# JediZ/PDE-based-image-processing

Hardware: AMD Instinct MI355X
Metric: SOR iterations/sec (3840x2160 flow) (higher is better)
Workload: dtype f32

## Files before the change

### include/pdeip.h

```cpp
#ifndef PDEIP_H
#define PDEIP_H

#ifdef __cplusplus
extern "C" {
#endif

#define PDEIP_OK 0
#define PDEIP_ERR_ARG 1
#define PDEIP_ERR_SOLVER 2
#define PDEIP_ERR_UNSUPPORTED 3
#define PDEIP_ERR_DEVICE 4
#define PDEIP_ERR_NOMEM 5

#define PDEIP_MODE_EXACT_ORDER 0
#define PDEIP_MODE_RED_BLACK 1
#define PDEIP_MODE_LINE_SCAN 2

#define PDEIP_SOLVER_SOR 1
#define PDEIP_SOLVER_ALR 2

const char *pdeip_version(void);
const char *pdeip_last_error(void);
int pdeip_set_mode(int mode);
int pdeip_get_mode(void);
int pdeip_set_device(int device_id);
int pdeip_set_devices(int n, const int *ids);
int pdeip_get_devices(int *ids, int capacity);
int pdeip_release(void);
int pdeip_last_launch_count(void);
int pdeip_workspace_generation(void);
int pdeip_persist_error(void);
int pdeip_debug_raise_abort(void);
int pdeip_debug_persist_order(int B, int T, int affine, int *table);
enum { PDEIP_PLAN_ELIN4 = 0, PDEIP_PLAN_LLIN4, PDEIP_PLAN_DISP4, PDEIP_PLAN_PDE4, PDEIP_PLAN_PDE8, PDEIP_PLAN_DISPSYM4 };
enum { PDEIP_PLAN_INFO = 11, PDEIP_PLAN_RECORD = 9 };
int pdeip_debug_plan_sor(int model, int nrows, int ncols, int nframes, int iter, int mode, int aligned16, int has_dst, int num_cus,
                         int rb2_slots, int rbp_slots, int *info, int *records, int capacity);
enum { PDEIP_PLAN_ALR_ELIN4 = 0, PDEIP_PLAN_ALR_LLIN4, PDEIP_PLAN_ALR_LLIN8, PDEIP_PLAN_ALR_DISP4, PDEIP_PLAN_ALR_PDE4, PDEIP_PLAN_ALR_PDE8 };
enum { PDEIP_PLAN_ALR_INFO = 12, PDEIP_PLAN_ALR_PASS = 20 };
int pdeip_debug_plan_alr(int model, int nrows, int ncols, int nframes, int iter, int mode, int *info, int *passes);
int pdeip_debug_rcp_check(unsigned long long *counts);
int pdeip_profile_enable(int on);
int pdeip_profile_read(double *elapsed_ms, int *sweep_launches);


int pdeip_oflow_sor_elin4(const float *U, const float *V, const float *M, const float *Cu,
                          const float *Cv, const float *Du, const float *Dv, const float *wW,
                          const float *wN, const float *wE, const float *wS, int nrows, int ncols,
                          int nframes_coef, int iter, float omega, int solver, float *U_out,
                          float *V_out, float *RU, float *RV);

int pdeip_oflow_sor_llin4(const float *U, const float *V, const float *dU, const float *dV,
                          const float *M, const float *Cu, const float *Cv, const float *Du,
                          const float *Dv, const float *wW, const float *wN, const float *wE,
                          const float *wS, int nrows, int ncols, int nframes_coef, int iter,
                          float omega, int solver, float *dU_out, float *dV_out, float *RU,
                          float *RV);

int pdeip_oflow_sor_llin8(const float *U, const float *V, const float *dU, const float *dV,
                          const float *M, const float *Cu, const float *Cv, const float *Du,
                          const float *Dv, const float *wW, const float *wNW, const float *wN,
                          const float *wNE, const float *wE, const float *wSE, const float *wS,
                          const float *wSW, int nrows, int ncols, int nframes_coef, int iter,
                          float omega, int solver, float *dU_out, float *dV_out, float *RU,
                          float *RV);

int pdeip_oflow_lhs_elin4(const float *U, const float *V, const float *M, const float *Du,
                          const float *Dv, const float *wW, const float *wN, const float *wE,
                          const float *wS, int nrows, int ncols, int nframes_coef, float *AU,
                          float *AV);

int pdeip_oflow_lhs_llin4(const float *U, const float *V, const float *dU, const float *dV,
                          const float *M, const float *Du, const float *Dv, const float *wW,
                          const float *wN, const float *wE, const float *wS, int nrows, int ncols,
                          int nframes_coef, float *AU, float *AV);

int pdeip_disp_sor_llin4(const float *U, const float *dU, const float *Cu, const float *Du,
                         const float *wW, const float *wN, const float *wE, const float *wS,
                         int nrows, int ncols, int iter, float omega, int solver, float *dU_out,
                         float *RU);

int pdeip_disp_sor_llin_sym4(const float *U0, const float *dU0, const float *Cu0, const float *Du0, const float *wW0,
// ... 409 lines not shown
```

### pde-based-image-processing_amd/capi.py

```python
import ctypes
import os

HERE = os.path.dirname(os.path.abspath(__file__))
LIB_PATH = os.environ.get("PDEIP_LIB") or os.path.join(HERE, "libpdeip.so")

PDEIP_OK = 0
PDEIP_ERR_ARG = 1
PDEIP_ERR_SOLVER = 2
PDEIP_ERR_UNSUPPORTED = 3
PDEIP_ERR_DEVICE = 4
PDEIP_ERR_NOMEM = 5
MODE_EXACT_ORDER = 0
MODE_RED_BLACK = 1
SEG_SURFACE, SEG_GREEDY, SEG_INVERSE = 0, 1, 2
MODE_LINE_SCAN = 2

_P = ctypes.c_void_p
_I = ctypes.c_int
_F = ctypes.c_float


class PdeipError(RuntimeError):

    def __init__(self, code, message):
# ... 113 lines not shown
                                 ctypes.c_ulonglong, _P, _P, _P, _P, _P],
    "pdeip_seg_label_dev": [_P, _P, _I, _I, _I, _P],
    "pdeip_seg_label": [_P, _I, _I, _I, _P],
    "pdeip_bwlabel_dev": [_P, _P, _I, _I, _I, _P, _P, _P, _I],
    "pdeip_bwlabel": [_P, _I, _I, _I, _P, _P, _P, _I],
    "pdeip_largest_component_dev": [_P, _P, _I, _I, _I, _F, _F, _P, _P, _P],
    "pdeip_largest_component": [_P, _I, _I, _I, _F, _F, _P, _P, _P],
    "pdeip_generate_seeds": [_P, _P, _I, _I, _I, ctypes.c_double, _P, _I, _I, _I, ctypes.c_double, ctypes.c_double, ctypes.c_ulonglong, _P, _P, _P,
                             _P, _P, _P],
    "pdeip_disp_segmentation": [_P, _I, _I, _P, _I, _P, _P, ctypes.c_ulonglong, _P, _P, _P, _P],
    "pdeip_nanmedfilt2_dev": [_P, _P, _I, _I, _I, _P],
    "pdeip_nanmedfilt2": [_P, _I, _I, _I, _P],
    "pdeip_sparse_pyramid": [_P, _I, _I, ctypes.c_double, ctypes.c_double, _I, _P, _P, _P],
    "pdeip_generate_seeds_sparse": [_P, _P, _I, _I, _I, ctypes.c_double, _P, _I, _I, _I, ctypes.c_double, ctypes.c_double, ctypes.c_ulonglong, _P,
                                    _P, _P, _P, _P, _P],
    "pdeip_region_competition_sparse": [_P, _P, _I, _I, _I, _I, _I, ctypes.c_double, _F, _I, ctypes.c_double, ctypes.c_double, ctypes.c_double,
                                        ctypes.c_ulonglong, _P, _P, _P, _P, _P],
    "pdeip_disp_segmentation_sparse": [_P, _I, _I, _P, _I, _P, _P, ctypes.c_ulonglong, _P, _P, _P, _P],
    "pdeip_flow2color_dev": [_P, _P, _P, _I, _I, ctypes.c_double, _I, _P, _P, _P],
    "pdeip_flow2color": [_P, _P, _I, _I, ctypes.c_double, _I, _P, _P, _P],
    "pdeip_flow_errors_dev": [_P, _P, _P, _P, _P, _P, _I, _I, _P, _P, _P],
    "pdeip_flow_errors": [_P, _P, _P, _P, _P, _I, _I, _P, _P, _P],
    "pdeip_disp_crosscheck_dev": [_P, _P, _P, _I, _I, ctypes.c_double, _P, _P, _P, _P],
    "pdeip_disp_crosscheck": [_P, _P, _I, _I, ctypes.c_double, _P, _P, _P, _P],
    "pdeip_flow_crosscheck_dev": [_P, _P, _P, _P, _P, _I, _I, ctypes.c_double, ctypes.c_double, _P, _P, _P],
    "pdeip_flow_crosscheck": [_P, _P, _P, _P, _I, _I, ctypes.c_double, ctypes.c_double, _P, _P, _P],
    "pdeip_nan_resize_dev": [_P, _P, _I, _I, _I, _I, _I, ctypes.c_double, _P],
    "pdeip_inpaint_meanfill_dev": [_P, _P, _I, _I, _I, _P],
    "pdeip_tv4_inpaint_assemble_dev": [_P, _P, _P, _P, _I, ctypes.c_double, _I, _I, _I, _F] + [_P] * 6,
    "pdeip_inpaint_merge_dev": [_P, _P, _P, _I, _I, _I, _P, _P],
    "pdeip_tv_inpaint4_dev": [_P, _P, _I, _I, _I, _P, _I, _P, _P, _P],
    "pdeip_tv_inpaint4": [_P, _I, _I, _I, _P, _I, _P, _P, _P],
    "pdeip_flow_splat_dev": [_P, _P, _P, _P, _P, _I, _I, _I, ctypes.c_double, _P, _P, _P],
    "pdeip_interp_blend_dev": [_P, _P, _P, _I, _P, _P, _P, _P, _I, _I, ctypes.c_double, _P, _P],
    "pdeip_flow_interpolate_dev": [_P, _P, _P, _I, _P, _P, _P, _P, _I, _I, ctypes.c_double, _P, _P, _P, _P, _P],
    "pdeip_flow_interpolate": [_P, _P, _I, _P, _P, _P, _P, _I, _I, ctypes.c_double, _P, _P, _P, _P, _P],
    "pdeip_gauss_taps": [ctypes.c_double, _P, _I, ctypes.POINTER(ctypes.c_int)],
    "pdeip_gauss": [_P, _I, _I, _I, ctypes.c_double, _P],
    "pdeip_gauss_dev": [_P, _P, _I, _I, _I, ctypes.c_double, _P],
    "pdeip_structure_tensor_dev": [_P, _P, _I, _I, _I, ctypes.c_double, ctypes.c_double, _P],
    "pdeip_st_weights_dev": [_P, _P, _I, _I, _P, ctypes.c_double, _P, _P],
    "pdeip_st_weights_padded_dev": [_P, _P, _I, _I, _P, ctypes.c_double, _P, _P],
    "pdeip_st_pad_dev": [_P, _P, _I, _I, _I, _P, _P],
    "pdeip_st_crop_dev": [_P, _P, _I, _I, _I, _P],
    "pdeip_diffusion8": [_P, _I, _I, _I, _P, _P],
    "pdeip_diffusion8_dev": [_P, _P, _I, _I, _I, _P, _P],
    "pdeip_set_mode": [_I],
    "pdeip_get_mode": [],
    "pdeip_set_device": [_I],
    "pdeip_set_devices": [_I, ctypes.POINTER(ctypes.c_int)],
    "pdeip_get_devices": [ctypes.POINTER(ctypes.c_int), _I],
    "pdeip_release": [],
    "pdeip_last_launch_count": [],
    "pdeip_workspace_generation": [],
    "pdeip_persist_error": [],
    "pdeip_debug_persist_order": [_I, _I, _I, ctypes.POINTER(ctypes.c_int)],
    "pdeip_debug_raise_abort": [],
    "pdeip_debug_plan_sor": [_I] * 11 + [ctypes.POINTER(ctypes.c_int), ctypes.POINTER(ctypes.c_int), _I],
    "pdeip_debug_plan_alr": [_I] * 6 + [ctypes.POINTER(ctypes.c_int), ctypes.POINTER(ctypes.c_int)],
    "pdeip_debug_rcp_check": [ctypes.POINTER(ctypes.c_ulonglong)],
    "pdeip_profile_enable": [_I],
    "pdeip_profile_read": [ctypes.POINTER(ctypes.c_double), ctypes.POINTER(ctypes.c_int)],
}
STRING_FUNCS = ("pdeip_version", "pdeip_last_error")

_lib = None


def load():
    global _lib
    if _lib is not None:
        return _lib
    if not os.path.exists(LIB_PATH):
        raise PdeipError(PDEIP_ERR_DEVICE,
                         "libpdeip.so is not built (%s). Run `python __graft_entry__.py build`; "
                         "there is no CPU fallback." % LIB_PATH)
    try:
        import torch
    except ImportError:
        pass
    try:
        lib = ctypes.CDLL(LIB_PATH)
    except OSError as exc:
        raise PdeipError(PDEIP_ERR_DEVICE, "cannot load %s: %s" % (LIB_PATH, exc)) from exc
    for name, argtypes in SIGNATURES.items():
        fn = getattr(lib, name)
        fn.argtypes = argtypes
        fn.restype = ctypes.c_int
    for name in STRING_FUNCS:
        fn = getattr(lib, name)
        fn.argtypes = []
        fn.restype = ctypes.c_char_p
    _lib = lib
    return lib


def last_error():
    return load().pdeip_last_error().decode("utf-8", "replace")


def check(rc):
    if rc != PDEIP_OK:
        raise PdeipError(rc, last_error())


_fn_cache = {}
# ... 43 lines not shown
```

### pde-based-image-processing_amd/csrc/pdeip_ctx.hip

```cpp
#include "pdeip_ctx.hpp"

namespace pdeip {

Context g;
thread_local ThreadState tls;

int set_err(int code, const char *fmt, ...)
{
    va_list ap;
    va_start(ap, fmt);
    vsnprintf(tls.err, sizeof tls.err, fmt, ap);
    va_end(ap);
    return code;
}

SweepTimer::SweepTimer(hipStream_t stream, int total_launches) : s(stream), total(total_launches)
{
    if (!g.profile) return;
    hipStreamCaptureStatus capturing = hipStreamCaptureStatusNone;
    if (hipStreamIsCapturing(s, &capturing) != hipSuccess || capturing != hipStreamCaptureStatusNone) return;
    std::lock_guard<std::mutex> lock(g.ev_mutex);
    if (g.n_ev >= Context::MAX_EV) return;
    if (g.n_ev == g.n_ev_created) {
        if (hipEventCreateWithFlags(&g.ev[g.n_ev][0], hipEventDisableSystemFence) != hipSuccess) return;
// ... 220 lines not shown
}

}

using namespace pdeip;

extern "C" const char *pdeip_version(void) { return "pdeip-mi355x 0.2 (gfx950)"; }
extern "C" const char *pdeip_last_error(void) { return tls.err; }
extern "C" int pdeip_set_mode(int mode)
{
    RC(check_mode("pdeip_set_mode", mode));
    g.mode = mode;
    mode_set_explicitly = true;
    return PDEIP_OK;
}
extern "C" int pdeip_get_mode(void)
{
    read_env_once();
    return g.mode;
}
extern "C" int pdeip_set_devices(int n, const int *ids)
{
    int have = 0;
    HIPCHK(hipGetDeviceCount(&have));
    if (n < 1 || n > MAX_DEVICES || !ids) return set_err(PDEIP_ERR_ARG, "pdeip_set_devices: need 1..%d device ids", MAX_DEVICES);
    for (int k = 0; k < n; k++) {
        if (ids[k] < 0 || ids[k] >= have || ids[k] >= MAX_DEVICES)
            return set_err(PDEIP_ERR_ARG, "pdeip_set_devices: no device %d (have %d)", ids[k], have);
        for (int j = 0; j < k; j++)
            if (ids[j] == ids[k]) return set_err(PDEIP_ERR_ARG, "pdeip_set_devices: device %d named twice", ids[k]);
    }
    for (int k = 0; k < n; k++) g.group[k] = ids[k];
    g.ngroup = n;
    devices_set_explicitly = true;
    return PDEIP_OK;
}
extern "C" int pdeip_set_device(int device_id) { return pdeip_set_devices(1, &device_id); }
extern "C" int pdeip_get_devices(int *ids, int capacity)
{
    read_env_once();
    for (int k = 0; k < g.ngroup && k < capacity; k++)
        if (ids) ids[k] = g.group[k];
    return g.ngroup;
}
extern "C" int pdeip_release(void)
{
    int cur = 0;
    const bool have_cur = hipGetDevice(&cur) == hipSuccess;
    for (int k = 0; k < MAX_DEVICES; k++) release_device(&g.devs[k]);
    if (have_cur) (void)hipSetDevice(cur);
    return PDEIP_OK;
}
extern "C" int pdeip_last_launch_count(void) { return tls.last_launches; }
extern "C" int pdeip_workspace_generation(void) { return g.ws_generation; }
extern "C" int pdeip_persist_error(void)
{
    bool bad = false;
    int cur = 0;
    const bool have_cur = hipGetDevice(&cur) == hipSuccess;
    for (int k = 0; k < MAX_DEVICES; k++) {
        DeviceState *d = &g.devs[k];
        if (d->device < 0) continue;
        if (d->persist_used && d->ws[WS_CTL]) {
            HIPCHK(hipSetDevice(d->device));
            unsigned word = 0;
            HIPCHK(hipDeviceSynchronize());
            HIPCHK(hipMemcpy(&word, d->ws[WS_CTL], sizeof word, hipMemcpyDeviceToHost));
            if (word != 0) {
                bad = true;
                HIPCHK(hipMemset(d->ws[WS_CTL], 0, sizeof(unsigned)));
            }
            d->persist_used = false;
        }
        if (d->abort_latched) bad = true;
        d->abort_latched = false;
    }
    if (have_cur) (void)hipSetDevice(cur);
    if (bad) return set_err(PDEIP_ERR_DEVICE, "persistent exact-order kernel: a dependency wait timed out (results are invalid)");
    return PDEIP_OK;
}
extern "C" int pdeip_debug_raise_abort(void)
{
    RC(use_device());
    float *ctl = nullptr;
    RC(ws_get(WS_CTL, 16, &ctl));
    const unsigned one = 1u;
    HIPCHK(hipDeviceSynchronize());
    HIPCHK(hipMemcpy(ctl, &one, sizeof one, hipMemcpyHostToDevice));
    cur_dev()->persist_used = true;
    return PDEIP_OK;
}

extern "C" int pdeip_profile_enable(int on)
{
    g.profile = (on != 0);
    g.n_ev = 0;
    return PDEIP_OK;
}
extern "C" int pdeip_profile_read(double *elapsed_ms, int *sweep_launches)
{
    double ms = 0.0;
    int launches = 0;
    for (int k = 0; k < g.n_ev; k++) {
        HIPCHK(hipEventSynchronize(g.ev[k][1]));
        float t = 0.0f;
        HIPCHK(hipEventElapsedTime(&t, g.ev[k][0], g.ev[k][1]));
// ... 9 lines not shown
```

### pde-based-image-processing_amd/csrc/pdeip_ctx.hpp

```cpp
#pragma once
#include "../../include/pdeip.h"

#include <hip/hip_runtime.h>
#include <hip/hip_ext.h>

#include <atomic>
#include <cstdarg>
#include <cstdio>
#include <cstdlib>
#include <cstring>
#include <map>
#include <mutex>
#include <vector>

namespace pdeip {

enum { WS_AUX0 = 0, WS_AUX1, WS_PING, WS_ARENA, WS_CTL, WS_ORDER, WS_ALR, WS_ALR_T, WS_TV, WS_SMALL, WS_MAIL, WS_PACK, WS_DRIVER, WS_LEX, WS_LS, WS_RANSAC, WS_SEG_STAGE, WS_SEG, WS_SEG_RC, WS_CCL, WS_SEEDS, WS_SELECT, WS_GAC, WS_RANSAC_BATCH, WS_FLOWVIZ, WS_CROSSCHECK, WS_INTERP, WS_GAUSS, WS_STENSOR, WS_NSLOT };

constexpr int MAX_DEVICES = 16;

struct DeviceState {
    int device = -1;
    void *ws[WS_NSLOT] = {};
    size_t ws_bytes[WS_NSLOT] = {};
    int num_cus = 0;
    bool persist_used = false;
    bool abort_latched = false;
    std::map<const void *, size_t> lds_opt_in;
    std::map<const void *, int> resident_waves;
    hipStream_t worker_stream = nullptr;
    void reset_caches()
    {
        persist_used = false;
    }
};

struct ThreadState {
    char err[512] = "";
    int last_launches = 0;
    int dev_slot = -1;
};
extern thread_local ThreadState tls;

struct Context {
    int mode = PDEIP_MODE_EXACT_ORDER;
    std::atomic<int> ws_generation{0};
    int rb_tj = 0;
    bool env_read = false;
    int ngroup = 1;
    int group[MAX_DEVICES] = {0};
    DeviceState devs[MAX_DEVICES];
    bool profile = false;
    static constexpr int MAX_EV = 4096;
    hipEvent_t ev[MAX_EV][2];
    int ev_launches[MAX_EV];
    int n_ev = 0, n_ev_created = 0;
    std::mutex ev_mutex;
};
extern Context g;

int set_err(int code, const char *fmt, ...);

#define HIPCHK(expr)                                                                                       \
    do {                                                                                                   \
        hipError_t e_ = (expr);                                                                            \
        if (e_ != hipSuccess) return ::pdeip::set_err(PDEIP_ERR_DEVICE, "%s failed: %s", #expr, hipGetErrorString(e_)); \
    } while (0)

#define RC(expr)             \
    do {                     \
        int rc_ = (expr);    \
        if (rc_) return rc_; \
    } while (0)

#define NONNULL(who, p)                                                                                \
    do {                                                                                               \
        if ((p) == nullptr) return ::pdeip::set_err(PDEIP_ERR_ARG, "%s: argument '%s' is NULL", who, #p); \
    } while (0)

struct SweepTimer {
    hipStream_t s;
    int slot = -1;
    int total = 0;
    explicit SweepTimer(hipStream_t stream, int total_launches = 0);
    hipEvent_t start_for(int launch) const { return (slot >= 0 && total > 0 && launch == 0) ? g.ev[slot][0] : nullptr; }
    hipEvent_t stop_for(int launch) const { return (slot >= 0 && total > 0 && launch == total - 1) ? g.ev[slot][1] : nullptr; }
    void stop(int launches);
};

template <class... KArgs, class... Args>
inline void launch_timed(void (*kernel)(KArgs...), dim3 grid, dim3 block, size_t lds, hipStream_t s, hipEvent_t start, hipEvent_t stop, Args... args)
{
// ... 45 lines not shown
```

### pde-based-image-processing_amd/csrc/pdeip_multi.hip

```cpp
#include "pdeip_ctx.hpp"

#include <thread>

using namespace pdeip;

namespace pdeip {

constexpr int OVERLAP_SLABS = 6;
struct SlabPlan {
    int nslabs = 1, halo = 0, nrows = 0;
    bool overlap = false;
    int c0[MAX_DEVICES], c1[MAX_DEVICES], lo[MAX_DEVICES], hi[MAX_DEVICES], dev[MAX_DEVICES];
};

int multi_plan(int ncols, int halo, SlabPlan *plan)
{
    read_env_once();
    int want = g.ngroup;
    const int virt = env_int("PDEIP_VIRTUAL_SLABS", 0);
    if (virt > want) want = virt;
    plan->overlap = false;
    if (want == 1 && virt <= 0 && env_int("PDEIP_HOST_OVERLAP", 1) != 0 && (long)ncols * plan->nrows >= (1L << 21) && ncols / OVERLAP_SLABS >= 4 * (halo + 1)) {
        want = OVERLAP_SLABS;
        plan->overlap = true;
// ... 98 lines not shown
    int vthreads = g.ngroup == 1 ? env_int("PDEIP_VIRTUAL_THREADS", plan.overlap ? 2 : 0) : 0;
    if (vthreads > plan.nslabs) vthreads = plan.nslabs;
    if (vthreads > MAX_DEVICES / 2) vthreads = MAX_DEVICES / 2;
    if (vthreads > 1) {
        nth = vthreads;
        for (int ti = 0; ti < nth; ti++) {
            devs[ti] = g.group[0];
            slot[ti] = ti == 0 ? -1 : MAX_DEVICES - ti;
        }
        for (int k = 0; k < plan.nslabs; k++) owner[k] = k % nth;
    } else {
        for (int k = 0; k < plan.nslabs; k++) {
            int j = 0;
            while (j < nth && devs[j] != plan.dev[k]) j++;
            if (j == nth) {
                devs[nth] = plan.dev[k];
                slot[nth++] = -1;
            }
            owner[k] = j;
        }
    }
    auto work = [&](int ti) {
        if (hipSetDevice(devs[ti]) != hipSuccess) {
            rc[ti] = PDEIP_ERR_DEVICE;
            snprintf(errs[ti], sizeof errs[ti], "multi-device call: hipSetDevice(%d) failed", devs[ti]);
            return;
        }
        const int keep_slot = tls.dev_slot;
        tls.dev_slot = slot[ti];
        DeviceState *ds = cur_dev();
        ds->device = devs[ti];
        if (ds->worker_stream == nullptr && hipStreamCreateWithFlags(&ds->worker_stream, hipStreamNonBlocking) != hipSuccess) {
            rc[ti] = PDEIP_ERR_DEVICE;
            snprintf(errs[ti], sizeof errs[ti], "multi-device call: cannot create a stream on device %d", devs[ti]);
            tls.dev_slot = keep_slot;
            return;
        }
        for (int k = 0; k < plan.nslabs && rc[ti] == PDEIP_OK; k++)
            if (owner[k] == ti) {
                rc[ti] = slab_run(mc, plan, k, ds->worker_stream);
                launches[ti] += tls.last_launches;
                if (rc[ti] != PDEIP_OK) snprintf(errs[ti], sizeof errs[ti], "%s", tls.err);
            }
        if (rc[ti] == PDEIP_OK && hipStreamSynchronize(ds->worker_stream) != hipSuccess) rc[ti] = PDEIP_ERR_DEVICE;
        tls.dev_slot = keep_slot;
    };
    if (nth == 1) work(0);
    else {
        for (int ti = 0; ti < nth; ti++) th[ti] = std::thread(work, ti);
        for (int ti = 0; ti < nth; ti++) th[ti].join();
    }
    (void)hipSetDevice(g.group[0]);
    tls.last_launches = 0;
    for (int ti = 0; ti < nth; ti++) tls.last_launches += launches[ti];
    for (int ti = 0; ti < nth; ti++)
        if (rc[ti] != PDEIP_OK) return set_err(rc[ti], "%s", errs[ti][0] ? errs[ti] : "multi-device call failed");
    return PDEIP_OK;
}

}
```

### pde-based-image-processing_amd/csrc/pdeip_sor5.hip

```cpp
#include "pdeip_ctx.hpp"

#include "pdeip_models.hpp"
#include "pdeip_pointwise.hpp"
#include "pdeip_sor_exact.hpp"
#include "pdeip_walk_host.hpp"
#include "pdeip_persist_host.hpp"
#include "pdeip_sor_rb.hpp"
#include "pdeip_sor_rbp.hpp"
#include "pdeip_sor_small.hpp"
#include "pdeip_sor_plan.hpp"

using namespace pdeip;

namespace {

constexpr int PS = RBP_SWEEPS;

template <class Mdl> SorTraits sor_traits()
{
    using PL = RbpLayout<Mdl, PS>;
    return SorTraits{Mdl::NIT, Mdl::NCF, false, 1, RB_OWN_ROWS, PL::FITS, PL::NW, RBP_OWN_ROWS, PL::nsteps(0), &SmallLayout<Mdl>::plan, &walk_width<Mdl>};
}

template <class Mdl> auto rb_kernel(bool vec, bool first, bool two)
// ... 72 lines not shown
    HIPCHK(hipGetLastError());
    return PDEIP_OK;
}

template <class Mdl> void bind_buffers(SweepPlanes<Mdl> &P, float *(&buf)[3][Mdl::NIT], const SorLaunch &l)
{
    for (int f = 0; f < Mdl::NIT; f++) {
        P.it_in[f] = buf[l.src][f];
        P.it_out[f] = buf[l.dst][f];
    }
}

template <class Mdl> int run_small(const SweepCall<Mdl> &c, const SorPlan &plan, float *(&buf)[3][Mdl::NIT])
{
    using SL = SmallLayout<Mdl>;
    const SmallPlan &sp = plan.small;
    SweepPlanes<Mdl> P = c.P;
    RC(ensure_lds(reinterpret_cast<const void *>(&k_sor_small<Mdl>), sp.lds));
    unsigned *counter = nullptr, *abort_word = nullptr;
    if (sp.nslabs > 1) {
        float *p = nullptr;
        RC(ws_get(WS_SMALL, 64, &p));
        counter = reinterpret_cast<unsigned *>(p);
        RC(ws_get(WS_CTL, 16, &p));
        abort_word = reinterpret_cast<unsigned *>(p);
    }
    DeviceState *d = cur_dev();
    SweepTimer timer(c.s);
    RC(for_each_launch(plan, [&](const SorLaunch &l) {
        bind_buffers<Mdl>(P, buf, l);
        const bool gated = sp.nslabs > 1 && l.src == l.dst;
        if (gated) d->persist_used = true;
        hipLaunchKernelGGL(k_sor_small<Mdl>, dim3((unsigned)sp.nslabs, (unsigned)c.nframes), dim3(SL::THREADS), sp.lds, c.s, P, c.nrows, c.ncols, l.sweeps,
                           c.omega, c.col0, c.n, sp.W, gated ? counter : nullptr, abort_word);
        tls.last_launches++;
        return PDEIP_OK;
    }));
    timer.stop(plan.nlaunch);
    HIPCHK(hipGetLastError());
    return PDEIP_OK;
}

#ifndef PDEIP_TIMER_MARKERS
#define PDEIP_TIMER_MARKERS 0
#endif

template <class Mdl> int run_chain(const SweepCall<Mdl> &c, const SorPlan &plan, float *(&buf)[3][Mdl::NIT])
{
    using PL = RbpLayout<Mdl, PS>;
    SweepPlanes<Mdl> P = c.P;
    hipStream_t s = c.s;
    SweepTimer timer(s, PDEIP_TIMER_MARKERS ? 0 : plan.nlaunch);
    int done = 0;
    RC(for_each_launch(plan, [&](const SorLaunch &l) {
        bind_buffers<Mdl>(P, buf, l);
        hipEvent_t const e0 = timer.start_for(l.index), e1 = timer.stop_for(l.index);
        if (l.kind == K_RBP) {
            RC(ensure_lds(reinterpret_cast<const void *>(rbp_kernel<Mdl>(l.first)), PL::LDS_BYTES));
            const bool keep = l.first && done + PS < c.iter;
            launch_timed(rbp_kernel<Mdl>(l.first), dim3((unsigned)l.gridx, (unsigned)c.nframes), dim3(PL::THREADS), PL::LDS_BYTES, s, e0, e1, P, keep ? c.aux0 : nullptr,
                         keep ? c.aux1 : nullptr, c.nrows, c.ncols, l.tj, l.tiles, l.units, c.omega, c.col0, c.n, plan.mirror_mode);
        } else {
            launch_timed(rb_kernel<Mdl>(plan.vec, l.first, l.sweeps == 2), dim3((unsigned)l.gridx, (unsigned)c.nframes), dim3(64 * RB_WAVES_PER_BLOCK), 0, s, e0, e1, P,
                         l.first ? c.aux0 : nullptr, l.first ? c.aux1 : nullptr, c.nrows, c.ncols, l.tj, l.tiles, l.units, c.omega, c.col0, c.n);
        }
        if (l.first) {
            P.cf[Mdl::D0] = c.aux0;
            P.cf[Mdl::D1] = c.aux1;
        }
        done += l.sweeps;
        tls.last_launches++;
        return PDEIP_OK;
    }));
    timer.stop(plan.nlaunch);
    if (plan.copy_back)
        for (int f = 0; f < Mdl::NIT; f++) RC(copy_d2d(s, buf[BUF_CALLER][f], buf[BUF_SCRATCH][f], c.n * c.nframes));
    HIPCHK(hipGetLastError());
    return PDEIP_OK;
}

template <class Mdl>
int run_sweeps(hipStream_t s, SweepPlanes<Mdl> P, int nrows, int ncols, int nframes, int iter,
               float omega, int mode, int col0, float *const *dst = nullptr)
{
    constexpr int NIT = Mdl::NIT;
    const size_t n = (size_t)nrows * ncols;
    tls.last_launches = 0;
    bool same = dst != nullptr, aligned = true;
    for (int f = 0; f < NIT; f++) {
        same = same && dst[f] == P.it_out[f];
        aligned = aligned && aligned16(P.it_out[f]) && (!dst || aligned16(dst[f]));
    }
    if (same) dst = nullptr;
    for (int f = 0; f < Mdl::NCF; f++) aligned = aligned && aligned16(P.cf[f]);
    for (int f = 0; f < Mdl::NRO; f++) aligned = aligned && aligned16(P.ro[f]);
    const SorShape sh{nrows, ncols, nframes, iter, mode, aligned, dst != nullptr, 0, 0};
    const SorPlan plan = plan_for<Mdl>(sh, SorDevice{});
    if (plan.copy_in)
        for (int f = 0; f < NIT; f++) RC(copy_d2d(s, dst[f], P.it_out[f], n * nframes));
    if (plan.family == SOR_NONE) return PDEIP_OK;
    SweepCall<Mdl> c{s, P, nrows, ncols, nframes, iter, omega, col0, n, nullptr, nullptr, dst};
    RC(ws_get(WS_AUX0, n * nframes * sizeof(float), &c.aux0));
    RC(ws_get(WS_AUX1, n * nframes * sizeof(float), &c.aux1));
    if (plan.family == SOR_EXACT) return run_exact(c, plan);
    float *scratch = nullptr;
    if (plan.family != SOR_SMALL) RC(ws_get(WS_PING, (size_t)NIT * n * nframes * sizeof(float), &scratch));
    float *buf[3][NIT];
    for (int f = 0; f < NIT; f++) {
        buf[BUF_CALLER][f] = P.it_out[f];
        buf[BUF_SCRATCH][f] = scratch ? scratch + (size_t)f * n * nframes : nullptr;
        buf[BUF_DST][f] = dst ? dst[f] : nullptr;
    }
    return plan.family == SOR_SMALL ? run_small(c, plan, buf) : run_chain(c, plan, buf);
}

}

extern "C" int pdeip_debug_plan_sor(int model, int nrows, int ncols, int nframes, int iter, int mode, int aligned16, int has_dst, int num_cus,
                                    int rb2_slots, int rbp_slots, int *info, int *records, int capacity)
{
    const char *who = "pdeip_debug_plan_sor";
    RC(check_dims(who, nrows, ncols, nframes));
    RC(check_mode(who, mode));
    if (info == nullptr || (records == nullptr && capacity > 0)) return set_err(PDEIP_ERR_ARG, "%s: null pointer", who);
    const SorShape sh{nrows, ncols, nframes, iter, mode, aligned16 != 0, has_dst != 0, 0, 0};
    const SorDevice dev{num_cus, rb2_slots, rbp_slots};
    SorPlan p;
    switch (model) {
    case PDEIP_PLAN_ELIN4: p = plan_for<ModelElin4>(sh, dev); break;
    case PDEIP_PLAN_LLIN4: p = plan_for<ModelLlin4>(sh, dev); break;
    case PDEIP_PLAN_DISP4: p = plan_for<ModelDisp4>(sh, dev); break;
    case PDEIP_PLAN_PDE4: p = plan_for<ModelPde4>(sh, dev); break;
    case PDEIP_PLAN_PDE8: p = plan_sor_pde8(sh, dev); break;
    case PDEIP_PLAN_DISPSYM4: p = plan_for<ModelDispSym4>(sh, dev); break;
    default: return set_err(PDEIP_ERR_ARG, "%s: unknown model %d", who, model);
    }
    const int head[PDEIP_PLAN_INFO] = {p.family, p.form, p.copy_back, p.copy_in, p.persist_setup, p.A, p.B, p.NC, p.W, p.last_m, 0};
    memcpy(info, head, sizeof head);
    for (int run = 0; run < (model == PDEIP_PLAN_DISPSYM4 ? 2 : 1); run++)
        (void)for_each_launch(p, [&](const SorLaunch &l) {
// ... 125 lines not shown
    float *const dst[2] = {dU_out, dV_out};
    RC(run_sweeps<ModelLlin4>(s, P, nrows, ncols, 1, iter, omega, mode, col0, dst));
    return PDEIP_OK;
}
extern "C" int pdeip_oflow_sor_llin4_dev(void *stream, const float *U, const float *V, float *dU, float *dV,
                                         const float *M, const float *Cu, const float *Cv, const float *Du,
                                         const float *Dv, const float *wW, const float *wN, const float *wE,
                                         const float *wS, int nrows, int ncols, int iter, float omega,
                                         int mode, int col0)
{
    return pdeip_oflow_sor_llin4_dev_to(stream, U, V, dU, dV, dU, dV, M, Cu, Cv, Du, Dv, wW, wN, wE, wS, nrows, ncols, iter, omega, mode, col0);
}

extern "C" int pdeip_disp_sor_llin4_dev_to(void *stream, const float *U, const float *dU, float *dU_out, const float *Cu,
                                           const float *Du, const float *wW, const float *wN, const float *wE, const float *wS,
                                           int nrows, int ncols, int iter, float omega, int mode, int col0)
{
    const char *who = "pdeip_disp_sor_llin4_dev";
    RC(check_dims(who, nrows, ncols, 1));
    RC(check_mode(who, mode));
    hipStream_t s = static_cast<hipStream_t>(stream);
    SweepPlanes<ModelDisp4> P{};
    P.it_out[0] = const_cast<float *>(dU);
    P.ro[0] = U;
    const float *cf[6] = {Cu, Du, wW, wN, wE, wS};
    for (int f = 0; f < 6; f++) P.cf[f] = cf[f];
    float *const dst[1] = {dU_out};
    RC(run_sweeps<ModelDisp4>(s, P, nrows, ncols, 1, iter, omega, mode, col0, dst));
    return PDEIP_OK;
}
extern "C" int pdeip_disp_sor_llin4_dev(void *stream, const float *U, float *dU, const float *Cu,
                                        const float *Du, const float *wW, const float *wN, const float *wE,
                                        const float *wS, int nrows, int ncols, int iter, float omega,
                                        int mode, int col0)
{
    return pdeip_disp_sor_llin4_dev_to(stream, U, dU, dU, Cu, Du, wW, wN, wE, wS, nrows, ncols, iter, omega, mode, col0);
}

extern "C" int pdeip_disp_sor_llin_sym4_dev(void *stream, const float *U0, float *dU0, const float *Cu0, const float *Du0,
                                            const float *wW0, const float *wN0, const float *wE0, const float *wS0,
                                            const float *U1, float *dU1, const float *Cu1, const float *Du1,
                                            const float *wW1, const float *wN1, const float *wE1, const float *wS1,
                                            int nrows, int ncols, int iter, float omega, int solver, int mode, int col0)
{
    const char *who = "pdeip_disp_sor_llin_sym4_dev";
    RC(check_dims(who, nrows, ncols, 1));
    RC(check_mode(who, mode));
    RC(check_solver(who, solver));
    hipStream_t s = static_cast<hipStream_t>(stream);
    if (iter <= 0) return PDEIP_OK;
    const float *U[2] = {U0, U1}, *cf[2][6] = {{Cu0, Du0, wW0, wN0, wE0, wS0}, {Cu1, Du1, wW1, wN1, wE1, wS1}};
    float *dU[2] = {dU0, dU1};
    int launches = 0;
    for (int k = 0; k < 2; k++) {
        if (solver == PDEIP_SOLVER_ALR) {
            RC(pdeip_disp_alr_llin4_dev(stream, U[k], dU[k], cf[k][0], cf[k][1], cf[k][2], cf[k][3], cf[k][4], cf[k][5], nrows, ncols, iter, omega, mode));
        } else {
            SweepPlanes<ModelDispSym4> P{};
            P.it_out[0] = dU[k];
            P.ro[0] = U[k];
            for (int f = 0; f < 6; f++) P.cf[f] = cf[k][f];
            RC(run_sweeps<ModelDispSym4>(s, P, nrows, ncols, 1, iter, omega, mode, col0));
        }
        launches += tls.last_launches;
    }
    tls.last_launches = launches;
    return PDEIP_OK;
}

extern "C" int pdeip_pde_sor4_dev_to(void *stream, const float *X, float *X_out, const float *TRACE, const float *B, const float *wW,
                                     const float *wN, const float *wE, const float *wS, int nrows, int ncols, int nframes, int iter,
                                     float omega, int mode, int col0)
{
    const char *who = "pdeip_pde_sor4_dev";
    RC(check_dims(who, nrows, ncols, nframes));
    RC(check_mode(who, mode));
    hipStream_t s = static_cast<hipStream_t>(stream);
    SweepPlanes<ModelPde4> P{};
    P.it_out[0] = const_cast<float *>(X);
    const float *cf[6] = {B, TRACE, wW, wN, wE, wS};
    for (int f = 0; f < 6; f++) P.cf[f] = cf[f];
    float *const dst[1] = {X_out};
    RC(run_sweeps<ModelPde4>(s, P, nrows, ncols, nframes, iter, omega, mode, col0, dst));
    return PDEIP_OK;
}
extern "C" int pdeip_pde_sor4_dev(void *stream, float *X, const float *TRACE, const float *B, const float *wW,
                                  const float *wN, const float *wE, const float *wS, int nrows, int ncols,
                                  int nframes, int iter, float omega, int mode, int col0)
{
    return pdeip_pde_sor4_dev_to(stream, X, X, TRACE, B, wW, wN, wE, wS, nrows, ncols, nframes, iter, omega, mode, col0);
}
```

### pde-based-image-processing_amd/csrc/pdeip_sor9.hip

```cpp
#include "pdeip_ctx.hpp"

#include "pdeip_models.hpp"
#include "pdeip_pointwise.hpp"
#include "pdeip_sor_pde8.hpp"
#include "pdeip_sor_pde8_persist.hpp"
#include "pdeip_persist_host.hpp"
#include "pdeip_sor_rb.hpp"
#include "pdeip_sor_plan.hpp"

using namespace pdeip;

namespace {

static_assert(P8_R == EX_R && P8_G == P8_SKEW + 1 && P8_H == P8_SKEW + 2, "plan_exact's fronts");
const SorTraits PDE8_TRAITS{1, ModelPde8::NCF, true, P8_SKEW, P8_OWN_ROWS2, false, 1, 1, 0, nullptr, nullptr};

auto p8_kernel(bool two, bool vec, bool first)
{
    static constexpr decltype(&k_pde8_colour<true, true>) table[2][2][2] = {
        {{&k_pde8_colour<false, false>, &k_pde8_colour<false, true>}, {&k_pde8_colour<true, false>, &k_pde8_colour<true, true>}},
        {{&k_pde8_colour2<false, false>, &k_pde8_colour2<false, true>}, {&k_pde8_colour2<true, false>, &k_pde8_colour2<true, true>}}};
    return table[two][vec][first];
}

// ... 36 lines not shown
        if (nl >= 0) timer.stop(nl);
    }
    if (nl < 0) return PDEIP_ERR_DEVICE;
    tls.last_launches += 1 + nl;
    HIPCHK(hipGetLastError());
    return PDEIP_OK;
}

int run_chain(const Pde8Call &c, const SorPlan &plan)
{
    const size_t nf = c.n * (size_t)c.nframes;
    float *buf[2] = {c.X, nullptr};
    RC(ws_get(WS_PING, nf * sizeof(float), &buf[BUF_SCRATCH]));
    Pde8SweepPlanes P{};
    for (int f = 0; f < ModelPde8::NCF; f++) P.cf[f] = c.cf[f];
    SweepTimer timer(c.s);
    RC(for_each_launch(plan, [&](const SorLaunch &l) {
        P.x_in = buf[l.src];
        P.x_out = buf[l.dst];
        hipLaunchKernelGGL(p8_kernel(l.sweeps == 2, plan.vec, l.first), dim3((unsigned)l.gridx, (unsigned)c.nframes), dim3(64 * RB_WAVES_PER_BLOCK), 0, c.s, P,
                           l.first ? c.bt : nullptr, l.first ? c.inv : nullptr, c.nrows, c.ncols, l.tj, l.tiles, l.units, c.omega, c.col0, c.n);
        if (l.first) {
            P.cf[ModelPde8::cB] = c.bt;
            P.cf[ModelPde8::cInv] = c.inv;
        }
        tls.last_launches++;
        return PDEIP_OK;
    }));
    timer.stop(plan.nlaunch);
    if (plan.copy_back) RC(copy_d2d(c.s, c.X, buf[BUF_SCRATCH], nf));
    HIPCHK(hipGetLastError());
    return PDEIP_OK;
}

}

SorPlan pdeip::plan_sor_pde8(SorShape sh, const SorDevice &dev)
{
    sh.has_dst = false;
    sh.packed_frame_bytes = pde8_pack_floats(sh.nrows, sh.ncols, 1) * sizeof(float);
    sh.persist_chunks = pde8_persist_chunks(sh.nrows);
    return plan_sor(PDE8_TRAITS, sh, dev, [](int) { return resident_waves(reinterpret_cast<const void *>(p8_kernel(true, true, false)), 64 * RB_WAVES_PER_BLOCK, RB_WAVES_PER_BLOCK); });
}

extern "C" int pdeip_pde_sor8_dev(void *stream, float *X, const float *TRACE, const float *B, const float *wW,
                                  const float *wNW, const float *wN, const float *wNE, const float *wE,
                                  const float *wSE, const float *wS, const float *wSW, int nrows, int ncols,
                                  int nframes, int iter, float omega, int mode, int col0)
{
    const char *who = "pdeip_pde_sor8_dev";
    RC(check_dims(who, nrows, ncols, nframes));
    RC(check_mode(who, mode));
    tls.last_launches = 0;
    Pde8Call c{static_cast<hipStream_t>(stream), X, {B, TRACE, wW, wNW, wN, wNE, wE, wSE, wS, wSW}, nullptr, nullptr, nrows, ncols, nframes, iter, omega, col0,
               (size_t)nrows * ncols};
    bool aligned = aligned16(X);
    for (int f = 0; f < ModelPde8::NCF; f++) aligned = aligned && aligned16(c.cf[f]);
    const SorPlan plan = plan_sor_pde8(SorShape{nrows, ncols, nframes, iter, mode, aligned, false, 0, 0}, SorDevice{});
    if (plan.family == SOR_NONE) return PDEIP_OK;
    RC(ws_get(WS_AUX0, c.n * nframes * sizeof(float), &c.bt));
    RC(ws_get(WS_AUX1, c.n * nframes * sizeof(float), &c.inv));
    return plan.family == SOR_EXACT ? run_exact(c, plan) : run_chain(c, plan);
}

#ifdef PDEIP_P8_STAMPS
extern "C" int pdeip_debug_read_p8_stamps(unsigned long long *out)
{
    HIPCHK(hipDeviceSynchronize());
    HIPCHK(hipMemcpyFromSymbol(out, HIP_SYMBOL(g_p8_stamps), 4096 * sizeof(unsigned long long)));
    return PDEIP_OK;
}
#endif
```

### pde-based-image-processing_amd/csrc/pdeip_sor_plan.hpp

```cpp
#pragma once
#include "pdeip_ctx.hpp"
#include "pdeip_sor_exact.hpp"
#include "pdeip_sor_rb.hpp"
#include "pdeip_sor_small.hpp"

namespace pdeip {

enum { SOR_NONE = 0, SOR_EXACT, SOR_SMALL, SOR_RB, SOR_RBP, SOR_PDE8 };
enum { FORM_NONE = 0, FORM_PERSIST, FORM_WALK, FORM_FRONT };
enum { K_RBP = 1, K_RB2, K_RB1, K_SMALL, K_P8C2, K_P8C1, K_PACK, K_PERSIST, K_WALK, K_DERIVE, K_FRONT, K_BORDERS };
enum { BUF_CALLER = 0, BUF_SCRATCH, BUF_DST };
constexpr int RBP_SWEEPS = 4;

struct SorTraits {
    int nit, ncf;
    bool pde8;
    int ex_skew;
    int rb2_own;
    bool rbp_fits;
    int rbp_nw, rbp_own, rbp_tail;
    SmallPlan (*small)(int, int, int, int);
    int (*walk_width)(int, int, int, int);
};
struct SorShape {
    int nrows, ncols, nframes, iter, mode;
    bool aligned16, has_dst;
    size_t packed_frame_bytes;
    int persist_chunks;
};
struct SorKnobs {
    bool persist = true, walk = false, small = true, fuse = true, pipe = true;
    int small_q = 1, rb_tj = 0, rbp_tj = 0, serpentine = 0;
};
struct SorDevice { int cus, rb2_slots, rbp_slots; };
enum { FACT_CUS, FACT_RB2, FACT_RBP };

struct SorLaunch { int kind, sweeps, first, tj, tiles, units, gridx, src, dst, count, index; };
struct SorPlan {
    int family = SOR_NONE, form = FORM_NONE;
    int A = 0, B = 0, NC = 0, W = 0, last_m = 0;
    int nsteps = 0, nlaunch = 0;
    SorLaunch step[4] = {};
    bool has_dst = false, vec = false;
    int mirror_mode = 0;
    bool copy_in = false;
    bool copy_back = false;
    bool persist_setup = false;
    SmallPlan small;
    void add(int kind, int count, int sweeps = 0, int tj = 0, int tiles = 0, int units = 0, int gridx = 0)
    {
        if (count <= 0) return;
        step[nsteps++] = SorLaunch{kind, sweeps, 0, tj, tiles, units, gridx, 0, 0, count, 0};
        nlaunch += count;
    }
};

enum { KNOBS_EXACT, KNOBS_SMALL, KNOBS_CHAIN, KNOBS_PIPE };
inline void read_sor_knobs(SorKnobs &k, int set, bool pde8 = false)
{
    if (set == KNOBS_EXACT) {
        k.persist = env_int(pde8 ? "PDEIP_PDE8_PERSIST" : "PDEIP_EXACT_PERSIST", 1) != 0;
        k.walk = !pde8 && k.persist && env_int("PDEIP_EXACT_WALK", 0) != 0;
    } else if (set == KNOBS_SMALL) {
        k.small = env_int("PDEIP_RB_SMALL", 1) != 0;
        if (k.small) k.small_q = env_int("PDEIP_SMALL_Q", 1);
    } else if (set == KNOBS_CHAIN) {
        static const bool fuse_enabled = env_int("PDEIP_RB_FUSE", 1) != 0;
        k.fuse = fuse_enabled;
        k.rb_tj = g.rb_tj > 0 ? g.rb_tj : env_int("PDEIP_RB_TJ", 0);
        k.pipe = !pde8 && env_int("PDEIP_RB_PIPE", 1) != 0;
    } else {
        k.rbp_tj = env_int("PDEIP_RBP_TJ", 0);
        const int serp = env_int("PDEIP_RBP_SERPENTINE", 0);
        k.serpentine = serp < 0 || serp > 2 ? 0 : serp;
    }
}

inline bool persist_fits(int strips, int iter, size_t plane_bytes, int ncols)
{
    return strips <= 0xffff && iter <= 0x7fff && plane_bytes < 0xffff0000ull && ncols <= 65535;
}

inline int pick_rb_tj(int forced) { return forced > 0 ? (forced < 2 ? 2 : forced) : 12; }

inline int pick_rb2_tj(int slots, int tiles, int ncols, int nframes)
{
    int best = 12;
    long best_cost = -1;
    for (int tj = 2; tj <= 64; tj++) {
        const long units = (long)tiles * ((ncols + tj - 1) / tj) * nframes;
        const long cost = ((units + slots - 1) / slots) * (tj + 6);
        if (best_cost < 0 || cost <= best_cost) {
            best_cost = cost;
            best = tj;
        }
    }
    return best;
}

inline int pick_rbp_tj(int slots, int tiles, int ncols, int nframes, int tail)
{
    int best = 64;
    long best_cost = -1;
    for (int tj = 8; tj <= 1024; tj++) {
        const long units = (long)tiles * ((ncols + tj - 1) / tj) * nframes;
        const long cost = ((units + slots - 1) / slots) * (tj + tail);
        if (best_cost < 0 || cost < best_cost) {
            best_cost = cost;
            best = tj;
        }
    }
    return best;
}

inline void plan_exact(SorPlan &p, const SorTraits &t, const SorShape &sh, const SorKnobs &k)
{
    const int skew = t.ex_skew;
    const int b64 = (sh.ncols - 2 + 63) / 64;
    const size_t n = (size_t)sh.nrows * sh.ncols;
    p.family = SOR_EXACT;
    p.copy_in = sh.has_dst;
    p.A = (sh.nrows - 2 + skew * 63 + EX_R - 1) / EX_R;
    p.last_m = (p.A - 1) + (skew + 1) * (b64 - 1) + (skew + 2) * (sh.iter - 1);
    const bool persist = k.persist && persist_fits(b64, sh.iter, n * (t.pde8 ? 1 : t.ncf) * sizeof(float), sh.ncols) && sh.packed_frame_bytes < 0xffff0000ull;
    p.W = persist && k.walk ? t.walk_width(sh.nrows, sh.ncols, sh.nframes, sh.iter) : 64;
    p.B = (sh.ncols - 2 + p.W - 1) / p.W;
    if (persist) {
// ... 1 lines not shown
        p.NC = sh.persist_chunks > 0 ? sh.persist_chunks : (sh.nrows - 2 + 63 + EX_CH - 1) / EX_CH;
        p.persist_setup = true;
        p.add(K_PACK, 1);
        p.add(k.walk ? K_WALK : K_PERSIST, 1, sh.iter, p.W, p.NC, p.B, p.B * sh.iter * sh.nframes);
    } else {
        p.form = FORM_FRONT;
        p.add(K_DERIVE, 1);
        p.add(K_FRONT, p.last_m + 1, 0, 64, p.A, p.B, p.B * sh.iter);
    }
    p.add(K_BORDERS, 1);
}

template <class Ask> inline bool plan_small(SorPlan &p, const SorTraits &t, const SorShape &sh, const SorKnobs &k, int cus, Ask &&ask)
{
    const int q = k.small_q < 1 ? 1 : k.small_q;
    SmallPlan sp = t.small(sh.nrows, sh.ncols, sh.iter, q);
    int per_launch = sh.iter;
    if (!sp.ok && sh.iter > SMALL_MAX_SWEEPS) {
        sp = t.small(sh.nrows, sh.ncols, SMALL_MAX_SWEEPS, q);
        per_launch = SMALL_MAX_SWEEPS;
    }
    if (sp.ok && sp.nslabs > 1 && cus <= 0) cus = ask(FACT_CUS);
    if (!sp.ok || (sp.nslabs > 1 && (long)sp.nslabs * sh.nframes > (long)cus - cus / 8)) return false;
    p.family = SOR_SMALL;
    p.small = sp;
    p.add(K_SMALL, sh.iter / per_launch, per_launch, sp.W, 1, sp.nslabs, sp.nslabs);
    p.add(K_SMALL, sh.iter % per_launch ? 1 : 0, sh.iter % per_launch, sp.W, 1, sp.nslabs, sp.nslabs);
    return true;
}

template <class Ask> inline void plan_chain(SorPlan &p, const SorTraits &t, const SorShape &sh, SorKnobs &k, const SorDevice &dev, Ask &&ask)
{
    const size_t n = (size_t)sh.nrows * sh.ncols;
    const auto strips = [&](int tj) { return (sh.ncols + tj - 1) / tj; };
    p.vec = sh.nrows % 4 == 0 && sh.aligned16;
    const bool pipe = k.pipe && k.fuse && p.vec && t.rbp_fits && (t.rbp_nw == 2 || n >= (size_t)1 << 21);
    const int n4 = pipe ? sh.iter / RBP_SWEEPS : 0, rest = sh.iter - RBP_SWEEPS * n4, n2 = k.fuse ? rest / 2 : 0, n1 = rest - 2 * n2;
    p.family = t.pde8 ? SOR_PDE8 : (n4 > 0 ? SOR_RBP : SOR_RB);
    if (n4 > 0) {
        read_sor_knobs(k, KNOBS_PIPE);
        const int tiles = (sh.nrows + t.rbp_own - 1) / t.rbp_own;
        const int tj = k.rbp_tj > 0 ? (k.rbp_tj < 2 ? 2 : k.rbp_tj)
                                    : pick_rbp_tj(dev.rbp_slots > 0 ? dev.rbp_slots : ask(FACT_RBP), tiles, sh.ncols, sh.nframes, t.rbp_tail);
        p.add(K_RBP, n4, RBP_SWEEPS, tj, tiles, tiles * strips(tj), tiles * strips(tj));
    }
    const int tj1 = pick_rb_tj(k.rb_tj), tiles1 = rb_row_tiles(sh.nrows, RB_OWN_ROWS), tiles2 = rb_row_tiles(sh.nrows, t.rb2_own);
    const int tj2 = (k.rb_tj > 0 || n2 == 0) ? tj1 : pick_rb2_tj(dev.rb2_slots > 0 ? dev.rb2_slots : ask(FACT_RB2), tiles2, sh.ncols, sh.nframes);
    const auto blocks = [](int units) { return (units + RB_WAVES_PER_BLOCK - 1) / RB_WAVES_PER_BLOCK; };
    p.add(t.pde8 ? K_P8C2 : K_RB2, n2, 2, tj2, tiles2, tiles2 * strips(tj2), blocks(tiles2 * strips(tj2)));
    p.add(t.pde8 ? K_P8C1 : K_RB1, n1, 1, tj1, tiles1, tiles1 * strips(tj1), blocks(tiles1 * strips(tj1)));
    p.copy_back = !sh.has_dst && (p.nlaunch & 1);
}

template <class Ask> inline SorPlan plan_sor(const SorTraits &t, const SorShape &sh, const SorDevice &dev, Ask &&ask)
{
    SorPlan p;
    SorKnobs k;
    p.has_dst = sh.has_dst;
    if (sh.iter <= 0) {
        p.copy_in = sh.has_dst;
    } else if (sh.mode != PDEIP_MODE_RED_BLACK) {
        read_sor_knobs(k, KNOBS_EXACT, t.pde8);
        plan_exact(p, t, sh, k);
    } else {
        if (!t.pde8) read_sor_knobs(k, KNOBS_SMALL);
        if (t.pde8 || !k.small || !plan_small(p, t, sh, k, dev.cus, ask)) {
            read_sor_knobs(k, KNOBS_CHAIN, t.pde8);
            plan_chain(p, t, sh, k, dev, ask);
            p.mirror_mode = k.serpentine;
        }
    }
    return p;
}

template <class F> inline int for_each_launch(const SorPlan &p, F &&fn)
{
    const int home = p.has_dst ? BUF_DST : BUF_CALLER;
    const auto out = [&](int i) -> int {
        if (p.family < SOR_RB) return home;
        if (p.has_dst) return ((p.nlaunch - 1 - i) & 1) ? BUF_SCRATCH : BUF_DST;
        return (i & 1) ? BUF_CALLER : BUF_SCRATCH;
    };
    int i = 0;
    for (int s = 0; s < p.nsteps; s++)
        for (int c = 0; c < p.step[s].count; c++, i++) {
            SorLaunch l = p.step[s];
            l.index = i;
            l.first = p.family != SOR_EXACT && i == 0;
            l.src = (i == 0 && p.family != SOR_EXACT) ? BUF_CALLER : out(i - 1);
            l.dst = out(i);
            RC(fn(l));
        }
    return PDEIP_OK;
}

SorPlan plan_sor_pde8(SorShape sh, const SorDevice &dev);

}
```

Before: 40860.

## Alternate RBP sweep direction across launches for large working sets

Adds a default mirror mode that alternates the traversal direction of successive pipelined red-black launches when the working set exceeds 256 MiB, so each launch starts where the previous one ended and can reuse data still resident in the last-level cache. The alternation state persists per device across calls. It also adds a debug API that records each launch's direction. The risk is that mirrored traversal has different access efficiency, and the state carried across calls makes the direction depend on call history.

```diff
diff --git a/include/pdeip.h b/include/pdeip.h
--- a/include/pdeip.h
+++ b/include/pdeip.h
@@ -28,6 +28,7 @@
 int pdeip_get_devices(int *ids, int capacity);
 int pdeip_release(void);
 int pdeip_last_launch_count(void);
+int pdeip_debug_last_directions(int *out, int cap);
 int pdeip_workspace_generation(void);
 int pdeip_persist_error(void);
 int pdeip_debug_raise_abort(void);
diff --git a/pde-based-image-processing_amd/capi.py b/pde-based-image-processing_amd/capi.py
--- a/pde-based-image-processing_amd/capi.py
+++ b/pde-based-image-processing_amd/capi.py
@@ -189,6 +189,7 @@
     "pdeip_get_devices": [ctypes.POINTER(ctypes.c_int), _I],
     "pdeip_release": [],
     "pdeip_last_launch_count": [],
+    "pdeip_debug_last_directions": [ctypes.POINTER(ctypes.c_int), _I],
     "pdeip_workspace_generation": [],
     "pdeip_persist_error": [],
     "pdeip_debug_persist_order": [_I, _I, _I, ctypes.POINTER(ctypes.c_int)],
diff --git a/pde-based-image-processing_amd/csrc/pdeip_ctx.hip b/pde-based-image-processing_amd/csrc/pdeip_ctx.hip
--- a/pde-based-image-processing_amd/csrc/pdeip_ctx.hip
+++ b/pde-based-image-processing_amd/csrc/pdeip_ctx.hip
@@ -296,6 +296,13 @@
     return PDEIP_OK;
 }
 extern "C" int pdeip_last_launch_count(void) { return tls.last_launches; }
+extern "C" int pdeip_debug_last_directions(int *out, int cap)
+{
+    const int n = (int)tls.last_directions.size();
+    for (int k = 0; k < n && k < cap; k++)
+        if (out) out[k] = tls.last_directions[k];
+    return n;
+}
 extern "C" int pdeip_workspace_generation(void) { return g.ws_generation; }
 extern "C" int pdeip_persist_error(void)
 {
diff --git a/pde-based-image-processing_amd/csrc/pdeip_ctx.hpp b/pde-based-image-processing_amd/csrc/pdeip_ctx.hpp
--- a/pde-based-image-processing_amd/csrc/pdeip_ctx.hpp
+++ b/pde-based-image-processing_amd/csrc/pdeip_ctx.hpp
@@ -29,6 +29,7 @@
     std::map<const void *, size_t> lds_opt_in;
     std::map<const void *, int> resident_waves;
     hipStream_t worker_stream = nullptr;
+    bool rbp_next_mirror = false;
     void reset_caches()
     {
         persist_used = false;
@@ -38,6 +39,7 @@
 struct ThreadState {
     char err[512] = "";
     int last_launches = 0;
+    std::vector<int> last_directions;
     int dev_slot = -1;
 };
 extern thread_local ThreadState tls;
diff --git a/pde-based-image-processing_amd/csrc/pdeip_multi.hip b/pde-based-image-processing_amd/csrc/pdeip_multi.hip
--- a/pde-based-image-processing_amd/csrc/pdeip_multi.hip
+++ b/pde-based-image-processing_amd/csrc/pdeip_multi.hip
@@ -174,6 +174,7 @@
     }
     (void)hipSetDevice(g.group[0]);
     tls.last_launches = 0;
+    tls.last_directions.clear();
     for (int ti = 0; ti < nth; ti++) tls.last_launches += launches[ti];
     for (int ti = 0; ti < nth; ti++)
         if (rc[ti] != PDEIP_OK) return set_err(rc[ti], "%s", errs[ti][0] ? errs[ti] : "multi-device call failed");
diff --git a/pde-based-image-processing_amd/csrc/pdeip_sor5.hip b/pde-based-image-processing_amd/csrc/pdeip_sor5.hip
--- a/pde-based-image-processing_amd/csrc/pdeip_sor5.hip
+++ b/pde-based-image-processing_amd/csrc/pdeip_sor5.hip
@@ -148,14 +148,16 @@
     hipStream_t s = c.s;
     SweepTimer timer(s, PDEIP_TIMER_MARKERS ? 0 : plan.nlaunch);
     int done = 0;
+    DeviceState *d = cur_dev();
     RC(for_each_launch(plan, [&](const SorLaunch &l) {
         bind_buffers<Mdl>(P, buf, l);
         hipEvent_t const e0 = timer.start_for(l.index), e1 = timer.stop_for(l.index);
+        const int mirror = l.kind == K_RBP ? resolve_mirror(plan.mirror_mode, d->rbp_next_mirror) : 0;
         if (l.kind == K_RBP) {
             RC(ensure_lds(reinterpret_cast<const void *>(rbp_kernel<Mdl>(l.first)), PL::LDS_BYTES));
             const bool keep = l.first && done + PS < c.iter;
             launch_timed(rbp_kernel<Mdl>(l.first), dim3((unsigned)l.gridx, (unsigned)c.nframes), dim3(PL::THREADS), PL::LDS_BYTES, s, e0, e1, P, keep ? c.aux0 : nullptr,
-                         keep ? c.aux1 : nullptr, c.nrows, c.ncols, l.tj, l.tiles, l.units, c.omega, c.col0, c.n, plan.mirror_mode);
+                         keep ? c.aux1 : nullptr, c.nrows, c.ncols, l.tj, l.tiles, l.units, c.omega, c.col0, c.n, mirror);
         } else {
             launch_timed(rb_kernel<Mdl>(plan.vec, l.first, l.sweeps == 2), dim3((unsigned)l.gridx, (unsigned)c.nframes), dim3(64 * RB_WAVES_PER_BLOCK), 0, s, e0, e1, P,
                          l.first ? c.aux0 : nullptr, l.first ? c.aux1 : nullptr, c.nrows, c.ncols, l.tj, l.tiles, l.units, c.omega, c.col0, c.n);
@@ -166,6 +168,7 @@
         }
         done += l.sweeps;
         tls.last_launches++;
+        tls.last_directions.push_back(mirror);
         return PDEIP_OK;
     }));
     timer.stop(plan.nlaunch);
@@ -182,6 +185,7 @@
     constexpr int NIT = Mdl::NIT;
     const size_t n = (size_t)nrows * ncols;
     tls.last_launches = 0;
+    tls.last_directions.clear();
     bool same = dst != nullptr, aligned = true;
     for (int f = 0; f < NIT; f++) {
         same = same && dst[f] == P.it_out[f];
@@ -413,6 +417,7 @@
     const float *U[2] = {U0, U1}, *cf[2][6] = {{Cu0, Du0, wW0, wN0, wE0, wS0}, {Cu1, Du1, wW1, wN1, wE1, wS1}};
     float *dU[2] = {dU0, dU1};
     int launches = 0;
+    std::vector<int> directions;
     for (int k = 0; k < 2; k++) {
         if (solver == PDEIP_SOLVER_ALR) {
             RC(pdeip_disp_alr_llin4_dev(stream, U[k], dU[k], cf[k][0], cf[k][1], cf[k][2], cf[k][3], cf[k][4], cf[k][5], nrows, ncols, iter, omega, mode));
@@ -422,10 +427,12 @@
             P.ro[0] = U[k];
             for (int f = 0; f < 6; f++) P.cf[f] = cf[k][f];
             RC(run_sweeps<ModelDispSym4>(s, P, nrows, ncols, 1, iter, omega, mode, col0));
+            directions.insert(directions.end(), tls.last_directions.begin(), tls.last_directions.end());
         }
         launches += tls.last_launches;
     }
     tls.last_launches = launches;
+    tls.last_directions = directions;
     return PDEIP_OK;
 }
 
diff --git a/pde-based-image-processing_amd/csrc/pdeip_sor9.hip b/pde-based-image-processing_amd/csrc/pdeip_sor9.hip
--- a/pde-based-image-processing_amd/csrc/pdeip_sor9.hip
+++ b/pde-based-image-processing_amd/csrc/pdeip_sor9.hip
@@ -112,6 +112,7 @@
     RC(check_dims(who, nrows, ncols, nframes));
     RC(check_mode(who, mode));
     tls.last_launches = 0;
+    tls.last_directions.clear();
     Pde8Call c{static_cast<hipStream_t>(stream), X, {B, TRACE, wW, wNW, wN, wNE, wE, wSE, wS, wSW}, nullptr, nullptr, nrows, ncols, nframes, iter, omega, col0,
                (size_t)nrows * ncols};
     bool aligned = aligned16(X);
diff --git a/pde-based-image-processing_amd/csrc/pdeip_sor_plan.hpp b/pde-based-image-processing_amd/csrc/pdeip_sor_plan.hpp
--- a/pde-based-image-processing_amd/csrc/pdeip_sor_plan.hpp
+++ b/pde-based-image-processing_amd/csrc/pdeip_sor_plan.hpp
@@ -11,6 +11,7 @@
 enum { K_RBP = 1, K_RB2, K_RB1, K_SMALL, K_P8C2, K_P8C1, K_PACK, K_PERSIST, K_WALK, K_DERIVE, K_FRONT, K_BORDERS };
 enum { BUF_CALLER = 0, BUF_SCRATCH, BUF_DST };
 constexpr int RBP_SWEEPS = 4;
+constexpr int MIRROR_ALTERNATE = 3;
 
 struct SorTraits {
     int nit, ncf;
@@ -71,8 +72,10 @@
         k.pipe = !pde8 && env_int("PDEIP_RB_PIPE", 1) != 0;
     } else {
         k.rbp_tj = env_int("PDEIP_RBP_TJ", 0);
-        const int serp = env_int("PDEIP_RBP_SERPENTINE", 0);
-        k.serpentine = serp < 0 || serp > 2 ? 0 : serp;
+        const char *serp = getenv("PDEIP_RBP_SERPENTINE");
+        const bool set = serp && *serp;
+        const int v = set ? atoi(serp) : 0;
+        k.serpentine = !set ? -1 : (v < 0 || v > MIRROR_ALTERNATE ? 0 : v);
     }
 }
 
@@ -180,6 +183,11 @@
     p.copy_back = !sh.has_dst && (p.nlaunch & 1);
 }
 
+inline int default_mirror(const SorShape &sh)
+{
+    return (size_t)13 * sh.nrows * sh.ncols * sh.nframes * sizeof(float) > ((size_t)256 << 20) ? MIRROR_ALTERNATE : 0;
+}
+
 template <class Ask> inline SorPlan plan_sor(const SorTraits &t, const SorShape &sh, const SorDevice &dev, Ask &&ask)
 {
     SorPlan p;
@@ -195,10 +203,17 @@
         if (t.pde8 || !k.small || !plan_small(p, t, sh, k, dev.cus, ask)) {
             read_sor_knobs(k, KNOBS_CHAIN, t.pde8);
             plan_chain(p, t, sh, k, dev, ask);
-            p.mirror_mode = k.serpentine;
+            p.mirror_mode = k.serpentine >= 0 ? k.serpentine : default_mirror(sh);
         }
     }
     return p;
+}
+
+inline int resolve_mirror(int mode, bool &next_mirror)
+{
+    const int m = mode == MIRROR_ALTERNATE ? (next_mirror ? 2 : 0) : mode;
+    next_mirror = m != 2;
+    return m;
 }
 
 template <class F> inline int for_each_launch(const SorPlan &p, F &&fn)
```

Result: faster. 46080 (median of 6 runs) (+12.8%).
